# FREDZEL2020/jittor-MYC-NeRFs

Measured on AMD Instinct MI355X. Metric: ray_samples_per_sec, higher is better.
Workload: dtype f32 (emulated: 3 x f16-split MFMA products, fp32 accumulate; fp32 VALU elsewhere); 1 GPU; TensorVMSplit 300^3 (16/48 comps, MLP_Fea 150-128-128-3), 800x800 rays x 512 samples/ray (BASELINE configs[1]); ONE frame per step at every N (N>1: split over the ranks, BASELINE configs[2]), 512-ray tiles round-robin, one RCCL all_gather of [4 cap] fp32 (rgb block + depth block, written in place by the render) + two strided un-permute copies; scene=synthetic scene A (SURVEY 8d), no alpha mask, white_bg, samples_per_ray=512, rays_per_rank=640000, tile=512, chunk=640000, alpha_mask=0, emulate_world=0, arith=f32

## Files before the change

jittor-myc-nerfs_amd/csrc/tvr_march.hip:

```cpp
#include <cstdlib>
#include "tvr_device.h"
#include "tvr_kernels.h"
#include "tvr_march_body.h"
#include "tvr_gradient.h"


template <bool DENSE, bool LDSL>
__global__ __launch_bounds__(64 * MARCH_MAX_WAVES) void march_kernel(const SceneDev sc, const float *__restrict__ rays,
                                                                     const int n_rays, const int S, const int s_cap,
                                                                     const MarchSampling sm, const float eps_T,
                                                                     MarchOut mo, const tvr_dense_out dn)
{
    constexpr bool CP = false, VOL = false;
    const CpDev cp = {};
    const float *const dvol = nullptr;
#include "tvr_march_body.inc"
}

template <bool DENSE, bool PLAIN>
__global__ __launch_bounds__(64 * MARCH_VOL_WAVES, DENSE ? MARCH_VOL_OCC - 1 : MARCH_VOL_OCC) void march_vol_kernel(const SceneDev sc, const float *__restrict__ dvol, const float *__restrict__ rays,
                                                                         const int n_rays, const int S, const int s_cap, const MarchSampling sm, const float eps_T,
                                                                         MarchOut mo, const tvr_dense_out dn)
{
    static_assert(!(PLAIN && DENSE), "the plain form has no dense outputs");
    constexpr bool LDSL = false, CP = false, VOL = true;
    const CpDev cp = {};
#include "tvr_march_body.inc"
}

__global__ __launch_bounds__(256) void density_volume_kernel(const SceneDev sc, float *__restrict__ out)
{
    const long long gx1 = sc.grid[0] + 1, gy1 = sc.grid[1] + 1, gz1 = sc.grid[2] + 1;
    const long long t = (long long)blockIdx.x * blockDim.x + threadIdx.x;
    if (t >= gx1 * gy1 * gz1) return;
    const long long x = t % gx1, y = (t / gx1) % gy1, z = t / (gx1 * gy1);
    const float4 *P[3] = {sc.dplane[0] + (y * gx1 + x) * 4, sc.dplane[1] + (z * gx1 + x) * 4, sc.dplane[2] + (z * gy1 + y) * 4};
    const float4 *Ln[3] = {sc.dline[0] + z * 4, sc.dline[1] + y * 4, sc.dline[2] + x * 4};
    double acc = 0.0;
#pragma unroll
    for (int i = 0; i < 3; ++i) {
#pragma unroll
        for (int g = 0; g < 4; ++g) {
            const float4 p = P[i][g], l = Ln[i][g];
            acc = acc + (double)p.x * (double)l.x;
            acc = acc + (double)p.y * (double)l.y;
            acc = acc + (double)p.z * (double)l.z;
            acc = acc + (double)p.w * (double)l.w;
        }
    }
    out[t] = (float)acc;
}

hipError_t launch_density_volume(const SceneDev &sc, float *out, hipStream_t stream)
{
    const long long n = ((long long)sc.grid[0] + 1) * ((long long)sc.grid[1] + 1) * ((long long)sc.grid[2] + 1);
    hipLaunchKernelGGL(density_volume_kernel, dim3((unsigned)((n + 255) / 256)), dim3(256), 0, stream, sc, out);
    return hipGetLastError();
}

#define COMP_LANES 8
__global__ __launch_bounds__(256) void composite_kernel(const MarchOut mo, const int n_rays, const int white_bg,
                                                        float *__restrict__ rgb_out)
{
    const int t = blockIdx.x * blockDim.x + threadIdx.x;
    const int r = t / COMP_LANES, l = t % COMP_LANES;
    const bool live = r < n_rays;
    const unsigned base = live ? mo.ray_off[r] : 0u, cnt = live ? mo.ray_cnt[r] : 0u;
    float c0 = 0.f, c1 = 0.f, c2 = 0.f;
    unsigned i = l;
    for (; i + 3 * COMP_LANES < cnt; i += 4 * COMP_LANES) {
        const float4 e0 = mo.q_out[base + i], e1 = mo.q_out[base + i + COMP_LANES], e2 = mo.q_out[base + i + 2 * COMP_LANES],
                     e3 = mo.q_out[base + i + 3 * COMP_LANES];
        c0 = c0 + e0.w * e0.x; c1 = c1 + e0.w * e0.y; c2 = c2 + e0.w * e0.z;
        c0 = c0 + e1.w * e1.x; c1 = c1 + e1.w * e1.y; c2 = c2 + e1.w * e1.z;
        c0 = c0 + e2.w * e2.x; c1 = c1 + e2.w * e2.y; c2 = c2 + e2.w * e2.z;
        c0 = c0 + e3.w * e3.x; c1 = c1 + e3.w * e3.y; c2 = c2 + e3.w * e3.z;
    }
    for (; i < cnt; i += COMP_LANES) {
        const float4 e = mo.q_out[base + i];
        c0 = c0 + e.w * e.x;
        c1 = c1 + e.w * e.y;
        c2 = c2 + e.w * e.z;
    }
#pragma unroll
    for (int off = 1; off < COMP_LANES; off <<= 1) {
        c0 = c0 + __shfl_xor(c0, off);
        c1 = c1 + __shfl_xor(c1, off);
        c2 = c2 + __shfl_xor(c2, off);
    }
    if (!live || l != 0) return;
    if (mo.counter[2] != 0u) {
        const float qnan = __int_as_float(0x7fc00000);
        rgb_out[(size_t)r * 3 + 0] = qnan; rgb_out[(size_t)r * 3 + 1] = qnan; rgb_out[(size_t)r * 3 + 2] = qnan;
        mo.depth[r] = qnan;
        return;
    }
    const float acc = mo.acc[r];
    if (white_bg) {
        const float bg = 1.0f - acc;
        c0 = c0 + bg; c1 = c1 + bg; c2 = c2 + bg;
    }
    rgb_out[(size_t)r * 3 + 0] = clamp01(c0);
    rgb_out[(size_t)r * 3 + 1] = clamp01(c1);
    rgb_out[(size_t)r * 3 + 2] = clamp01(c2);
}

__global__ __launch_bounds__(256) void scatter_rgb_kernel(const MarchOut mo, const int S, float *__restrict__ rgb_dense)
{
    const unsigned n = *mo.counter;
    for (unsigned e = blockIdx.x * blockDim.x + threadIdx.x; e < n; e += gridDim.x * blockDim.x) {
        const float4 v = mo.q_out[e];
        const size_t q = ((size_t)mo.q_ray[e] * S + mo.q_j[e]) * 3;
        rgb_dense[q] = v.x; rgb_dense[q + 1] = v.y; rgb_dense[q + 2] = v.z;
    }
}

__global__ __launch_bounds__(256) void density_feature_kernel(const SceneDev sc, const float *__restrict__ xyz, const long long m,
                                                              float *__restrict__ out)
{
    const long long t = (long long)blockIdx.x * blockDim.x + threadIdx.x;
    const long long s = t >> 2;
    const int sub = threadIdx.x & 3;
    float part = 0.0f;
    if (s < m) {
        int i0[3];
        float w[3];
#pragma unroll
        for (int k = 0; k < 3; ++k) {
            const float f = unnorm(xyz[s * 3 + k], sc.gm1[k]);
            const float fl = floorf(fminf(fmaxf(f, -2.0f), sc.gm1[k] + 2.0f));
            i0[k] = (int)fl;
            w[k] = f - fl;
        }
        const float4 a = vm_term<4, true>(sc.dplane[0], sc.dline[0], sc.grid[0], sc.grid[1], sc.grid[2], i0[0], i0[1], i0[2], w[0], w[1], w[2], sub);
        const float4 b = vm_term<4, true>(sc.dplane[1], sc.dline[1], sc.grid[0], sc.grid[2], sc.grid[1], i0[0], i0[2], i0[1], w[0], w[2], w[1], sub);
        const float4 c = vm_term<4, true>(sc.dplane[2], sc.dline[2], sc.grid[1], sc.grid[2], sc.grid[0], i0[1], i0[2], i0[0], w[1], w[2], w[0], sub);
        part = ((a.x + a.y) + (a.z + a.w)) + ((b.x + b.y) + (b.z + b.w)) + ((c.x + c.y) + (c.z + c.w));
    }
    part += __shfl_xor(part, 1);
    part += __shfl_xor(part, 2);
    if (s < m && sub == 0) out[s] = part;
}

__global__ __launch_bounds__(256) void density_gradient_kernel(const SceneDev sc, const float *__restrict__ xyz, const long long m, const float3 h, const float3 inv2h,
                                                               float *__restrict__ sigma_feature, float *__restrict__ grad)
{
    const long long t = (long long)blockIdx.x * blockDim.x + threadIdx.x;
    const long long s = t >> 2;
    const int sub = threadIdx.x & 3;
    float f[7];
#pragma unroll
    for (int j = 0; j < 7; ++j) f[j] = 0.0f;
    if (s < m) vm_grad_point(sc, xyz[s * 3], xyz[s * 3 + 1], xyz[s * 3 + 2], h, sub, f);
#pragma unroll
    for (int j = 0; j < 7; ++j) {
        f[j] += __shfl_xor(f[j], 1);
        f[j] += __shfl_xor(f[j], 2);
    }
    if (s < m && sub == 0) {
        if (sigma_feature) sigma_feature[s] = f[0];
        grad[s * 3 + 0] = (f[1] - f[2]) * inv2h.x;
        grad[s * 3 + 1] = (f[3] - f[4]) * inv2h.y;
        grad[s * 3 + 2] = (f[5] - f[6]) * inv2h.z;
    }
}

__global__ __launch_bounds__(256) void alpha_sample_kernel(const SceneDev sc, const float *__restrict__ xyz, const long long m,
                                                           float *__restrict__ out)
{
    const long long s = (long long)blockIdx.x * blockDim.x + threadIdx.x;
    if (s >= m) return;
    const float p[3] = {xyz[s * 3], xyz[s * 3 + 1], xyz[s * 3 + 2]};
    out[s] = alpha_lookup(sc, p);
}

__global__ __launch_bounds__(256) void alpha_bits_kernel(const float *__restrict__ vol, const long long n, unsigned *__restrict__ bits)
{
    const long long wd = (long long)blockIdx.x * blockDim.x + threadIdx.x;
    if (wd * 32 >= n) return;
    unsigned v = 0u;
    for (int b = 0; b < 32; ++b) {
        const long long i = wd * 32 + b;
        if (i < n && vol[i] > 0.0f) v |= 1u << b;
    }
    bits[wd] = v;
}

hipError_t launch_alpha_bits(const float *vol, long long n, unsigned *bits, hipStream_t stream)
{
    const long long words = (n + 31) / 32;
    hipLaunchKernelGGL(alpha_bits_kernel, dim3((unsigned)((words + 255) / 256)), dim3(256), 0, stream, vol, n, bits);
    return hipGetLastError();
}

template <bool DENSE, bool LDSL>
static hipError_t launch_march_t(const SceneDev &sc, const float *rays, int n_rays, int S, const MarchSampling &sm, float eps_T, const MarchOut &mo,
                                 const tvr_dense_out &dn, int waves, size_t lds, unsigned grid, hipStream_t stream)
{
    hipError_t rc = hipFuncSetAttribute((const void *)march_kernel<DENSE, LDSL>, hipFuncAttributeMaxDynamicSharedMemorySize, (int)lds);
    if (rc != hipSuccess) return rc;
    hipLaunchKernelGGL((march_kernel<DENSE, LDSL>), dim3(grid), dim3(64 * waves), lds, stream, sc, rays, n_rays, S, S, sm, eps_T, mo, dn);
    return hipGetLastError();
}

static int device_cu_count()
{
    static int cus = 0;
    if (cus == 0) {
        int dev = 0, n = 0;
        if (hipGetDevice(&dev) == hipSuccess && hipDeviceGetAttribute(&n, hipDeviceAttributeMultiprocessorCount, dev) == hipSuccess && n > 0) cus = n;
        else cus = 256;
    }
    return cus;
}

int march_cu_count() { return device_cu_count(); }

static hipError_t launch_march_vol(const SceneDev &sc, const float *dvol, const float *rays, int n_rays, int S, const MarchSampling &sm, float eps_T, const MarchOut &mo,
                                   const tvr_dense_out *dense, hipStream_t stream)
{
    const int groups = MARCH_VOL_GROUPS;
    const size_t kLds = 160 * 1024 / (size_t)groups, per_wave = (size_t)S * 6, fixed = MARCH_HDR + 64;
    int waves = (int)((kLds - fixed) / per_wave);
    waves = waves >= MARCH_VOL_WAVES ? MARCH_VOL_WAVES : (waves >= 8 ? 8 : (waves >= 4 ? 4 : (waves >= 2 ? 2 : 1)));
    const size_t lds = fixed + (size_t)waves * per_wave;
    const int n_tiles = (n_rays + MARCH_TILE - 1) / MARCH_TILE;
    long long grid = (long long)device_cu_count() * groups * (MARCH_VOL_WAVES / waves);
    if (grid > n_tiles) grid = n_tiles;
    if (grid < 1) grid = 1;
    tvr_dense_out none = {};
    const tvr_dense_out &dn = dense ? *dense : none;
    const unsigned long long vol_bytes = 4ull * (unsigned long long)(sc.grid[0] + 1) * (unsigned long long)(sc.grid[1] + 1) * (unsigned long long)(sc.grid[2] + 1);
    const bool plain = !dense && sc.avol == nullptr && sm.zv == nullptr && mo.lam6 == nullptr && vol_bytes < (1ull << 32);
    const void *fn = dense ? (const void *)march_vol_kernel<true, false> : (plain ? (const void *)march_vol_kernel<false, true> : (const void *)march_vol_kernel<false, false>);
    hipError_t rc = hipFuncSetAttribute(fn, hipFuncAttributeMaxDynamicSharedMemorySize, (int)lds);
    if (rc != hipSuccess) return rc;
    if (dense) hipLaunchKernelGGL((march_vol_kernel<true, false>), dim3((unsigned)grid), dim3(64 * waves), lds, stream, sc, dvol, rays, n_rays, S, S, sm, eps_T, mo, dn);
    else if (plain) hipLaunchKernelGGL((march_vol_kernel<false, true>), dim3((unsigned)grid), dim3(64 * waves), lds, stream, sc, dvol, rays, n_rays, S, S, sm, eps_T, mo, dn);
    else hipLaunchKernelGGL((march_vol_kernel<false, false>), dim3((unsigned)grid), dim3(64 * waves), lds, stream, sc, dvol, rays, n_rays, S, S, sm, eps_T, mo, dn);
    return hipGetLastError();
}

hipError_t launch_march(const SceneDev &sc, const float *rays, int n_rays, int S, const MarchSampling &sm, float eps_T,
                        const MarchOut &mo, const tvr_dense_out *dense, hipStream_t stream, const float *dvol)
{
    if (dvol) return launch_march_vol(sc, dvol, rays, n_rays, S, sm, eps_T, mo, dense, stream);
    const size_t kLds = 160 * 1024, line_bytes = ((size_t)sc.grid[0] + sc.grid[1] + sc.grid[2] + 3) * 16 * MARCH_LSTRIDE, per_wave = (size_t)S * 6;
    bool ldsl = MARCH_HDR + line_bytes + 4 * per_wave + 64 <= kLds;
    const size_t fixed = MARCH_HDR + (ldsl ? line_bytes : 0) + 64;
    int waves = (int)((kLds - fixed) / per_wave);
    waves = waves >= 16 ? 16 : (waves >= 12 ? 12 : (waves >= 8 ? 8 : (waves >= 4 ? 4 : (waves >= 2 ? 2 : 1))));
    const size_t lds = fixed + (size_t)waves * per_wave;
    const int n_tiles = (n_rays + MARCH_TILE - 1) / MARCH_TILE;
    long long grid = (long long)device_cu_count() * (16 / waves > 0 ? 16 / waves : 1);
    if (grid > n_tiles) grid = n_tiles;
    if (grid < 1) grid = 1;
    tvr_dense_out none = {};
    const tvr_dense_out &dn = dense ? *dense : none;
    if (dense) return ldsl ? launch_march_t<true, true>(sc, rays, n_rays, S, sm, eps_T, mo, dn, waves, lds, (unsigned)grid, stream)
                           : launch_march_t<true, false>(sc, rays, n_rays, S, sm, eps_T, mo, dn, waves, lds, (unsigned)grid, stream);
    return ldsl ? launch_march_t<false, true>(sc, rays, n_rays, S, sm, eps_T, mo, dn, waves, lds, (unsigned)grid, stream)
                : launch_march_t<false, false>(sc, rays, n_rays, S, sm, eps_T, mo, dn, waves, lds, (unsigned)grid, stream);
}

hipError_t launch_composite(const MarchOut &mo, int n_rays, int white_bg, float *rgb, hipStream_t stream)
{
    const long long threads = (long long)n_rays * COMP_LANES;
    hipLaunchKernelGGL(composite_kernel, dim3((unsigned)((threads + 255) / 256)), dim3(256), 0, stream, mo, n_rays, white_bg, rgb);
    return hipGetLastError();
}

hipError_t launch_scatter_rgb(const MarchOut &mo, int S, float *rgb_dense, hipStream_t stream)
{
    hipLaunchKernelGGL(scatter_rgb_kernel, dim3(1024), dim3(256), 0, stream, mo, S, rgb_dense);
    return hipGetLastError();
}

hipError_t launch_density_feature(const SceneDev &sc, const float *xyz, long long m, float *out, hipStream_t stream)
{
    const long long blocks = (m * 4 + 255) / 256;
    hipLaunchKernelGGL(density_feature_kernel, dim3((unsigned)blocks), dim3(256), 0, stream, sc, xyz, m, out);
    return hipGetLastError();
}

hipError_t launch_density_gradient(const SceneDev &sc, const float *xyz, long long m, const float h[3], const float inv2h[3], float *sigma_feature, float *grad,
                                   hipStream_t stream)
{
    const long long blocks = (m * 4 + 255) / 256;
    hipLaunchKernelGGL(density_gradient_kernel, dim3((unsigned)blocks), dim3(256), 0, stream, sc, xyz, m, make_float3(h[0], h[1], h[2]),
                       make_float3(inv2h[0], inv2h[1], inv2h[2]), sigma_feature, grad);
    return hipGetLastError();
}

hipError_t launch_alpha_sample(const SceneDev &sc, const float *xyz, long long m, float *out, hipStream_t stream)
{
    hipLaunchKernelGGL(alpha_sample_kernel, dim3((unsigned)((m + 255) / 256)), dim3(256), 0, stream, sc, xyz, m, out);
    return hipGetLastError();
}
```

jittor-myc-nerfs_amd/csrc/tvr_march_body.h:

```cpp
#pragma once
#include "tvr_device.h"
#include "tvr_kernels.h"

#define MARCH_MAX_WAVES 16
#define MARCH_TILE 16
#define MARCH_SPIN_LIMIT (1u << 22)
#define MARCH_SLOTS 64u
#ifndef MARCH_CTR_WORD
#define MARCH_CTR_WORD 1
#endif
#ifndef MARCH_TAIL
#define MARCH_TAIL 4u
#endif
#ifndef MARCH_VOL_WAVES
#define MARCH_VOL_WAVES 16
#endif
#ifndef MARCH_VOL_GROUPS
#define MARCH_VOL_GROUPS 1
#endif
#ifndef MARCH_VOL_OCC
#define MARCH_VOL_OCC 8
#endif
#define MARCH_HDR 560
#ifndef MARCH_LSTRIDE
#define MARCH_LSTRIDE 4
#endif

__device__ __forceinline__ float4 vm_term_lds(const float4 *__restrict__ P, const float4 *Ls, int W, int x0, int y0, int l0,
                                              float wx, float wy, float wl, int sub)
{
    const float ux = 1.0f - wx, uy = 1.0f - wy, ul = 1.0f - wl;
    const int Wp = W + 1;
    const unsigned cell = __umul24((unsigned)y0, (unsigned)Wp) + (unsigned)x0;
    unsigned o0 = (cell << 6) + ((unsigned)sub << 4), o1 = o0 + ((unsigned)Wp << 6);
    asm volatile("" : "+v"(o0), "+v"(o1));
    const unsigned char *pb = (const unsigned char *)P;
    const float4 t00 = *(const float4 *)(pb + (size_t)o0), t01 = *(const float4 *)(pb + (size_t)o0 + 64);
    const float4 t10 = *(const float4 *)(pb + (size_t)o1), t11 = *(const float4 *)(pb + (size_t)o1 + 64);
    const float4 *q = Ls + l0 * MARCH_LSTRIDE + sub;
    const float4 l0v = q[0], l1v = q[MARCH_LSTRIDE];
    float4 p4 = f4_mul(ux * uy, t00);
    p4 = f4_fma(wx * uy, t01, p4);
    p4 = f4_fma(ux * wy, t10, p4);
    p4 = f4_fma(wx * wy, t11, p4);
    float4 q4 = f4_mul(ul, l0v);
    q4 = f4_fma(wl, l1v, q4);
    return make_float4(p4.x * q4.x, p4.y * q4.y, p4.z * q4.z, p4.w * q4.w);
}

__device__ __forceinline__ float cp_density_quad(const SceneDev &sc, const CpDev &cp, int ix, int iy, int iz, float wx, float wy, float wz, int sub)
{
    const int tpt = cp.rd >> 2;
    const float4 *__restrict__ l0 = sc.dline[0] + (size_t)iz * tpt + sub;
    const float4 *__restrict__ l1 = sc.dline[1] + (size_t)iy * tpt + sub;
    const float4 *__restrict__ l2 = sc.dline[2] + (size_t)ix * tpt + sub;
    const float ux = 1.0f - wx, uy = 1.0f - wy, uz = 1.0f - wz;
    float part = 0.0f;
    for (int g = 0; g < tpt; g += 4) {
        const float4 a0 = l0[g], a1 = l0[g + tpt], b0 = l1[g], b1 = l1[g + tpt], c0 = l2[g], c1 = l2[g + tpt];
        const float4 a = f4_fma(wz, a1, f4_mul(uz, a0)), b = f4_fma(wy, b1, f4_mul(uy, b0)), c = f4_fma(wx, c1, f4_mul(ux, c0));
        const float tx = (a.x * b.x) * c.x, ty = (a.y * b.y) * c.y, tz = (a.z * b.z) * c.z, tw = (a.w * b.w) * c.w;
        part = part + ((tx + ty) + (tz + tw));
    }
    return part;
}

struct __attribute__((packed, aligned(4))) vol_pair { float a, b; };
__device__ __forceinline__ float vol_density(const float *__restrict__ D, int gx1, int gy1, int ix, int iy, int iz, float wx, float wy, float wz)
{
    const size_t sy = (size_t)gx1, sz = (size_t)gx1 * (size_t)gy1;
    const float *r = D + ((size_t)iz * sz + (size_t)iy * sy + (size_t)ix);
    const vol_pair p00 = *(const vol_pair *)r, p01 = *(const vol_pair *)(r + sy);
    const vol_pair p10 = *(const vol_pair *)(r + sz), p11 = *(const vol_pair *)(r + sz + sy);
    const float c00 = __builtin_fmaf(wx, p00.b - p00.a, p00.a), c01 = __builtin_fmaf(wx, p01.b - p01.a, p01.a);
    const float c10 = __builtin_fmaf(wx, p10.b - p10.a, p10.a), c11 = __builtin_fmaf(wx, p11.b - p11.a, p11.a);
    const float c0 = __builtin_fmaf(wy, c01 - c00, c00), c1 = __builtin_fmaf(wy, c11 - c10, c10);
    return __builtin_fmaf(wz, c1 - c0, c0);
}

constexpr bool PLAIN = false;

struct MarchVolArgs {
    SceneDev sc;
    const float *dvol, *rays;
    int n_rays, S, s_cap;
    MarchSampling sm;
    float eps_T;
    MarchOut mo;
    tvr_dense_out dn;
};
template <bool ON_DEMAND, typename T>
__device__ __forceinline__ T march_arg_now(const T &arg, unsigned offset)
{
#if defined(__HIP_DEVICE_COMPILE__)
    if constexpr (ON_DEMAND) {
        const __attribute__((address_space(4))) unsigned char *ka = (const __attribute__((address_space(4))) unsigned char *)__builtin_amdgcn_kernarg_segment_ptr();
        asm volatile("" : "+s"(ka));
        return *(const __attribute__((address_space(4))) T *)(ka + offset);
    }
#endif
    return arg;
}

__device__ __forceinline__ float vol_density32(const unsigned char *r00, const unsigned char *r01, const unsigned char *r10, const unsigned char *r11, unsigned gx1,
                                               unsigned gy1, int ix, int iy, int iz, float wx, float wy, float wz)
{
    const unsigned row = __umul24((unsigned)iz, gy1) + (unsigned)iy;
    unsigned o = (row * gx1 + (unsigned)ix) << 2;
    asm volatile("" : "+v"(o));
    const vol_pair p00 = *(const vol_pair *)(r00 + (size_t)o), p01 = *(const vol_pair *)(r01 + (size_t)o);
    const vol_pair p10 = *(const vol_pair *)(r10 + (size_t)o), p11 = *(const vol_pair *)(r11 + (size_t)o);
    const float c00 = __builtin_fmaf(wx, p00.b - p00.a, p00.a), c01 = __builtin_fmaf(wx, p01.b - p01.a, p01.a);
    const float c10 = __builtin_fmaf(wx, p10.b - p10.a, p10.a), c11 = __builtin_fmaf(wx, p11.b - p11.a, p11.a);
    const float c0 = __builtin_fmaf(wy, c01 - c00, c00), c1 = __builtin_fmaf(wy, c11 - c10, c10);
    return __builtin_fmaf(wz, c1 - c0, c0);
}

#ifndef MARCH_VOL_LEAN
#define MARCH_VOL_LEAN 1
#endif
__device__ __forceinline__ float march_expf(float x)
{
    const float p = x * 0x1.715476p+0f;
    const float r = __builtin_rintf(p);
    float lo = __builtin_fmaf(x, 0x1.715476p+0f, -p);
    lo = __builtin_fmaf(x, 0x1.4ae0bep-26f, lo);
    return __builtin_ldexpf(__builtin_amdgcn_exp2f((p - r) + lo), (int)r);
}
__device__ __forceinline__ float march_softplus(float x)
{
    if (x > 20.0f) return x;
    const float t = march_expf(x);
    const float u = 1.0f + t, d = u - 1.0f;
    const float rc = __builtin_amdgcn_rcpf(d);
    float q = t * rc;
    q = __builtin_fmaf(__builtin_fmaf(-d, q, t), rc, q);
    const float lg = __builtin_amdgcn_logf(u) * 0x1.62e430p-1f;
    return d == 0.0f ? t : lg * q;
}

#define MARCH_DPP_WAVE_SHR1 0x138
#define MARCH_DPP_SAME 0xE4
template <int CTRL, int ROWS>
__device__ __forceinline__ float march_dpp_mov(float old, float v)
{
    return __int_as_float(__builtin_amdgcn_update_dpp(__float_as_int(old), __float_as_int(v), CTRL, ROWS, 0xF, false));
}
template <int N>
__device__ __forceinline__ float march_up(float v)
{
    float t = march_dpp_mov<MARCH_DPP_WAVE_SHR1, 0xF>(1.0f, v);
#pragma unroll
    for (int i = 1; i < N; ++i) t = march_dpp_mov<MARCH_DPP_WAVE_SHR1, 0xF>(t, t);
    return t;
}
__device__ __forceinline__ void scan_mul_dpp(float &x, float &excl, float &last)
{
    x = x * march_up<1>(x);
    x = x * march_up<2>(x);
    x = x * march_up<4>(x);
    x = x * march_up<8>(x);
    {
        const auto q = __builtin_amdgcn_permlane16_swap(__float_as_uint(x), __float_as_uint(x), false, false);
        const auto s = __builtin_amdgcn_permlane32_swap(q[0], q[1], false, false);
        float t = march_dpp_mov<MARCH_DPP_SAME, 0x6>(1.0f, __uint_as_float(s[0]));
        t = march_dpp_mov<MARCH_DPP_SAME, 0x8>(t, __uint_as_float(q[0]));
        x = x * t;
    }
    {
        const auto h = __builtin_amdgcn_permlane32_swap(__float_as_uint(x), __float_as_uint(x), false, false);
        x = x * march_dpp_mov<MARCH_DPP_SAME, 0xC>(1.0f, __uint_as_float(h[0]));
    }
    excl = march_up<1>(x);
    last = __int_as_float(__builtin_amdgcn_readlane(__float_as_int(x), 63));
}
```

jittor-myc-nerfs_amd/csrc/tvr_march_body.inc:

```
    static_assert(!(CP && LDSL), "the CP lines (up to 96 channels) do not go through LDS");
    static_assert(!(VOL && (CP || LDSL)), "the baked volume replaces the factored evaluation: no lines in LDS, no CP lines");
    extern __shared__ __attribute__((aligned(16))) unsigned char lds_raw[];
    const int lane = threadIdx.x & 63;
    const int wave = __builtin_amdgcn_readfirstlane(threadIdx.x >> 6);
    const int n_waves = blockDim.x >> 6;
    unsigned *cursor = (unsigned *)lds_raw;
    const float4 *ls0 = (const float4 *)(lds_raw + MARCH_HDR);
    const int ln0 = LDSL ? (sc.grid[2] + 1) * MARCH_LSTRIDE : 0, ln1 = LDSL ? (sc.grid[1] + 1) * MARCH_LSTRIDE : 0, ln2 = LDSL ? (sc.grid[0] + 1) * MARCH_LSTRIDE : 0;
    const float4 *ls1 = ls0 + ln0, *ls2 = ls1 + ln1;
    float *bufw = (float *)(ls2 + ln2) + (size_t)wave * s_cap;
    unsigned short *bufj = (unsigned short *)((float *)(ls2 + ln2) + (size_t)n_waves * s_cap) + (size_t)wave * s_cap;
#ifdef TVR_MARCH_TIMELINE
    unsigned long long tl_chunks = 0ull, tl_rays = 0ull;
    if (mo.stats && threadIdx.x == 0) mo.stats[32 + 8 * blockIdx.x] = __builtin_amdgcn_s_memrealtime();
#endif
    if (threadIdx.x == 0) *cursor = 0u;
    unsigned long long *slots = (unsigned long long *)(lds_raw + 16);
    if (threadIdx.x < MARCH_SLOTS) slots[threadIdx.x] = 0ull;
    unsigned long long *gstat = (unsigned long long *)(lds_raw + 16 + 8 * MARCH_SLOTS);
    if (threadIdx.x < 3) gstat[threadIdx.x] = 0ull;
    if (LDSL) {
        float4 *dst = (float4 *)(lds_raw + MARCH_HDR);
        for (int i = threadIdx.x; i < (sc.grid[2] + 1) * 4; i += blockDim.x) dst[(i >> 2) * MARCH_LSTRIDE + (i & 3)] = sc.dline[0][i];
        for (int i = threadIdx.x; i < (sc.grid[1] + 1) * 4; i += blockDim.x) dst[ln0 + (i >> 2) * MARCH_LSTRIDE + (i & 3)] = sc.dline[1][i];
        for (int i = threadIdx.x; i < (sc.grid[0] + 1) * 4; i += blockDim.x) dst[ln0 + ln1 + (i >> 2) * MARCH_LSTRIDE + (i & 3)] = sc.dline[2][i];
    }
    __syncthreads();
#ifdef TVR_MARCH_TIMELINE
    if (mo.stats && threadIdx.x == 0) mo.stats[32 + 8 * blockIdx.x + 1] = __builtin_amdgcn_s_memrealtime();
#endif
    const int sub = lane & 3;
    const unsigned char *vrow[4] = {nullptr, nullptr, nullptr, nullptr};
    if constexpr (PLAIN) {
        const size_t vsy = (size_t)(sc.grid[0] + 1) * 4, vsz = vsy * (size_t)(sc.grid[1] + 1);
        vrow[0] = (const unsigned char *)dvol; vrow[1] = vrow[0] + vsy; vrow[2] = vrow[0] + vsz; vrow[3] = vrow[2] + vsy;
    }
    unsigned long long clk0 = 0ull, ref0 = 0ull;
    if (march_arg_now<PLAIN>(mo.stats, offsetof(MarchVolArgs, mo.stats)) && threadIdx.x == 0) { clk0 = __builtin_amdgcn_s_memtime(); ref0 = __builtin_amdgcn_s_memrealtime(); }

    unsigned long long st_eval = 0, st_bbox = 0, st_term = 0;
    int last_start = 0;

    for (;;) {
        unsigned ci = 0;
        if (lane == 0) ci = atomicAdd(cursor, 1u);
        ci = __builtin_amdgcn_readfirstlane(ci);
        int ray_start, ray_len;
        {
            const unsigned k = ci / MARCH_TILE, slot = k & (MARCH_SLOTS - 1u);
            if ((ci % MARCH_TILE) == 0u) {
                unsigned t = 0, len = MARCH_TILE;
                if (lane == 0) {
                    if ((long long)n_rays >= 8LL * MARCH_TILE * (long long)gridDim.x && (long long)last_start + 2LL * MARCH_TILE * (long long)gridDim.x >= (long long)n_rays)
                        len = MARCH_TAIL;
                    t = atomicAdd(march_arg_now<PLAIN>(mo.counter, offsetof(MarchVolArgs, mo.counter)) + MARCH_CTR_WORD, len);
                    const unsigned long long genw = (unsigned long long)(k + 1u) | (len == MARCH_TAIL ? 0x80000000ull : 0ull);
#ifdef TVR_FAULT_INJECT_MARCH
                    if (blockIdx.x == 0 && k == 3u) __hip_atomic_store(&slots[slot], ((unsigned long long)(k + 1u + MARCH_SLOTS) << 32) | t, __ATOMIC_RELEASE, __HIP_MEMORY_SCOPE_WORKGROUP);
                    else
#endif
                    __hip_atomic_store(&slots[slot], (genw << 32) | t, __ATOMIC_RELEASE, __HIP_MEMORY_SCOPE_WORKGROUP);
                }
                ray_start = (int)__builtin_amdgcn_readfirstlane(t);
                ray_len = (int)__builtin_amdgcn_readfirstlane(len);
            } else {
                unsigned long long v;
                unsigned spins = 0u, fault = 0u;
                for (;;) {
                    v = __hip_atomic_load(&slots[slot], __ATOMIC_ACQUIRE, __HIP_MEMORY_SCOPE_WORKGROUP);
                    const unsigned gen = (unsigned)(v >> 32) & 0x7fffffffu;
                    if (gen == k + 1u) break;
                    if (gen > k + 1u) { fault = 1u; break; }
                    if (++spins > MARCH_SPIN_LIMIT) { fault = 2u; break; }
                    __builtin_amdgcn_s_sleep(1);
                }
                if (fault) {
                    if (lane == 0) atomicOr(march_arg_now<PLAIN>(mo.counter, offsetof(MarchVolArgs, mo.counter)) + 2, fault);
                    break;
                }
                ray_start = (int)(unsigned)v;
                ray_len = (v >> 63) ? MARCH_TAIL : MARCH_TILE;
            }
        }
        if (ray_start >= n_rays) break;
        if ((int)(ci % MARCH_TILE) >= ray_len) continue;
        last_start = ray_start;
        const int ray = ray_start + (int)(ci % MARCH_TILE);
        if (ray >= n_rays) continue;
        const float *__restrict__ const rays_r = march_arg_now<PLAIN>(rays, offsetof(MarchVolArgs, rays));
        const float *const jit_r = march_arg_now<PLAIN>(sm.jitter, offsetof(MarchVolArgs, sm.jitter));
        float o[3], d[3];
#pragma unroll
        for (int k = 0; k < 3; ++k) {
            o[k] = rays_r[(size_t)ray * 6 + k];
            d[k] = rays_r[(size_t)ray * 6 + 3 + k];
        }
        const float tmin = ray_tmin(sc, o, d);
        const bool has_jit = jit_r != nullptr;
        const float u = has_jit ? jit_r[ray] : 0.0f;
        const float *__restrict__ zrow = (!PLAIN && sm.zv) ? sm.zv + (size_t)ray * S : nullptr;
        float lam6 = 1.0f;
        int n6 = 0;

        float T = 1.0f, acc_l = 0.0f, dep_l = 0.0f;
        int napp = 0;
        bool seen = false, terminated = false;
        int c = 0;
        for (; c * 64 < S; ++c) {
            const int j = c * 64 + lane;
            const bool inr = j < S;
            float fj = (float)j, fj1 = (float)(j + 1);
            if (has_jit) { fj = fj + u; fj1 = fj1 + u; }
            float z = tmin + sc.step * fj;
            float z1 = tmin + sc.step * fj1;
            if (zrow) {
                z = inr ? zrow[j] : 0.0f;
                z1 = (j < S - 1) ? zrow[j + 1] : z;
            }
            float p[3], n[3], f[3];
            bool bbox = inr;
#pragma unroll
            for (int k = 0; k < 3; ++k) {
                p[k] = o[k] + d[k] * z;
                bbox = bbox & !((sc.lo[k] > p[k]) | (p[k] > sc.hi[k]));
            }
            bool valid = bbox;
            if (!PLAIN && sc.avol != nullptr) {
                if (bbox) valid = sc.abits ? alpha_positive(sc, p) : (alpha_lookup(sc, p) > 0.0f);
            }
            int i0[3];
            float w[3];
#pragma unroll
            for (int k = 0; k < 3; ++k) {
                n[k] = (p[k] - sc.lo[k]) * sc.inv[k] - 1.0f;
                f[k] = unnorm(n[k], sc.gm1[k]);
                const float fl = floorf(f[k]);
                i0[k] = (int)fl;
                w[k] = f[k] - fl;
            }
            if constexpr (PLAIN) asm volatile("" : "+v"(i0[0]), "+v"(i0[1]), "+v"(i0[2]), "+v"(w[0]), "+v"(w[1]), "+v"(w[2]));
            const unsigned long long mb = __ballot(bbox), mv = __ballot(valid);
            if (DENSE) {
                const size_t q = (size_t)ray * S + j;
                if (inr) {
                    if (dn.z) dn.z[q] = z;
                    if (dn.valid) dn.valid[q] = valid;
                    if (dn.bbox_valid) dn.bbox_valid[q] = bbox;
                    if (dn.cell) { dn.cell[q * 3] = i0[0]; dn.cell[q * 3 + 1] = i0[1]; dn.cell[q * 3 + 2] = i0[2]; }
                }
            }
            st_bbox += __popcll(mb);
            if (mv == 0ull) {
                if (DENSE && inr) {
                    const size_t q = (size_t)ray * S + j;
                    if (dn.sigma_feature) dn.sigma_feature[q] = 0.f;
                    if (dn.sigma) dn.sigma[q] = 0.f;
                    if (dn.alpha) dn.alpha[q] = 0.f;
                    if (dn.weight) dn.weight[q] = 0.f;
                }
                if (mb == 0ull && seen && !DENSE) break;
                continue;
            }
            seen = true;
            st_eval += __popcll(mv);
#ifdef TVR_MARCH_TIMELINE
            tl_chunks++;
#endif

            float sf = 0.0f;
            if constexpr (VOL) {
                if constexpr (PLAIN) {
                    if (valid) sf = vol_density32(vrow[0], vrow[1], vrow[2], vrow[3], (unsigned)(sc.grid[0] + 1), (unsigned)(sc.grid[1] + 1), i0[0], i0[1], i0[2], w[0], w[1], w[2]);
                } else
                if (valid) sf = vol_density(dvol, sc.grid[0] + 1, sc.grid[1] + 1, i0[0], i0[1], i0[2], w[0], w[1], w[2]);
            } else {
#pragma unroll
                for (int k4 = 0; k4 < 4; ++k4) {
                    const bool v = quad_bcast_i((int)valid, k4) != 0;
                    if (__ballot(v) == 0ull) continue;
                    const int ix = quad_bcast_i(i0[0], k4), iy = quad_bcast_i(i0[1], k4), iz = quad_bcast_i(i0[2], k4);
                    const float wx = quad_bcast_f(w[0], k4), wy = quad_bcast_f(w[1], k4), wz = quad_bcast_f(w[2], k4);
                    float part = 0.0f;
                    if constexpr (CP) {
                        if (v) part = cp_density_quad(sc, cp, ix, iy, iz, wx, wy, wz, sub);
                    } else
                    if (v && LDSL) {
                        const float4 a = vm_term_lds(sc.dplane[0], ls0, sc.grid[0], ix, iy, iz, wx, wy, wz, sub);
                        const float4 b = vm_term_lds(sc.dplane[1], ls1, sc.grid[0], ix, iz, iy, wx, wz, wy, sub);
                        const float4 cc = vm_term_lds(sc.dplane[2], ls2, sc.grid[1], iy, iz, ix, wy, wz, wx, sub);
                        part = ((a.x + a.y) + (a.z + a.w)) + ((b.x + b.y) + (b.z + b.w)) + ((cc.x + cc.y) + (cc.z + cc.w));
                    } else if (v) {
                        const float4 a = vm_term<4, false>(sc.dplane[0], sc.dline[0], sc.grid[0], sc.grid[1], sc.grid[2], ix, iy, iz, wx, wy, wz, sub);
                        const float4 b = vm_term<4, false>(sc.dplane[1], sc.dline[1], sc.grid[0], sc.grid[2], sc.grid[1], ix, iz, iy, wx, wz, wy, sub);
                        const float4 cc = vm_term<4, false>(sc.dplane[2], sc.dline[2], sc.grid[1], sc.grid[2], sc.grid[0], iy, iz, ix, wy, wz, wx, sub);
                        part = ((a.x + a.y) + (a.z + a.w)) + ((b.x + b.y) + (b.z + b.w)) + ((cc.x + cc.y) + (cc.z + cc.w));
                    }
                    part += quad_perm_f<QUAD_XOR1>(part);
                    part += quad_perm_f<QUAD_XOR2>(part);
                    if (sub == k4) sf = part;
                }
            }

            float sigma = 0.0f;
            constexpr bool LEAN = VOL && MARCH_VOL_LEAN;
            if constexpr (LEAN) {
                if (valid) sigma = (sc.act == 0) ? march_softplus(sf + sc.shift) : fmaxf(sf, 0.0f);
            } else
            if (valid) sigma = (sc.act == 0) ? softplus_f(sf + sc.shift) : fmaxf(sf, 0.0f);
            float dist = (j < S - 1) ? (z1 - z) : 0.0f;
            dist = dist * sc.scale;
            const float alpha = 1.0f - (LEAN ? march_expf(-sigma * dist) : expf(-sigma * dist));
            const float fT = (1.0f - alpha) + 1e-10f;
            if (!PLAIN && mo.lam6) {
                float f6 = inr ? (1.0f - alpha) + 1e-6f : 1.0f;
#pragma unroll
                for (int off = 32; off > 0; off >>= 1) f6 = f6 * __shfl_xor(f6, off);
                lam6 = lam6 * f6;
                n6 += min(64, S - c * 64);
            }
            float incl = fT, excl, last;
            if constexpr (VOL) {
                scan_mul_dpp(incl, excl, last);
            } else {
#pragma unroll
                for (int off = 1; off < 64; off <<= 1) {
                    const float t = __shfl_up(incl, off);
                    if (lane >= off) incl = incl * t;
                }
                excl = __shfl_up(incl, 1);
                if (lane == 0) excl = 1.0f;
            }
            const float Tj = T * excl;
            const float wgt = alpha * Tj;
            acc_l += wgt;
            dep_l += wgt * z;
            const bool app = wgt > sc.thres;
            const unsigned long long ma = __ballot(app);
            if (ma) {
                const int pos = napp + __popcll(ma & ((1ull << lane) - 1ull));
                if (app) { bufw[pos] = wgt; bufj[pos] = (unsigned short)j; }
                napp += __popcll(ma);
            }
            if constexpr (VOL) T = T * last;
            else T = T * __shfl(incl, 63);
            if (DENSE && inr) {
                const size_t q = (size_t)ray * S + j;
                if (dn.sigma_feature) dn.sigma_feature[q] = valid ? sf : 0.f;
                if (dn.sigma) dn.sigma[q] = sigma;
                if (dn.alpha) dn.alpha[q] = alpha;
                if (dn.weight) dn.weight[q] = wgt;
            }
            if (T < eps_T) { terminated = true; ++c; break; }
        }
        if (DENSE) {
            for (int cc = c; cc * 64 < S; ++cc) {
                const int j = cc * 64 + lane;
                if (j < S) {
                    const size_t q = (size_t)ray * S + j;
                    const float fjj = has_jit ? ((float)j + u) : (float)j;
                    if (dn.z) dn.z[q] = zrow ? zrow[j] : tmin + sc.step * fjj;
                    if (dn.valid) dn.valid[q] = 0;
                    if (dn.bbox_valid) dn.bbox_valid[q] = 0;
                    if (dn.cell) { dn.cell[q * 3] = 0; dn.cell[q * 3 + 1] = 0; dn.cell[q * 3 + 2] = 0; }
                    if (dn.sigma_feature) dn.sigma_feature[q] = 0.f;
                    if (dn.sigma) dn.sigma[q] = 0.f;
                    if (dn.alpha) dn.alpha[q] = 0.f;
                    if (dn.weight) dn.weight[q] = 0.f;
                }
            }
        }
        st_term += terminated ? 1 : 0;
#ifdef TVR_MARCH_TIMELINE
        tl_rays++;
#endif

        const float acc = wave_sum(acc_l);
        const float dep = wave_sum(dep_l);
        const MarchOut mt = march_arg_now<PLAIN>(mo, offsetof(MarchVolArgs, mo));
        unsigned base = 0;
        if (lane == 0 && napp > 0) base = atomicAdd(mt.counter, (unsigned)napp);
        base = __shfl(base, 0);
        if (lane == 0) {
            mt.ray_off[ray] = base;
            mt.ray_cnt[ray] = (unsigned)napp;
            mt.acc[ray] = acc;
            mt.depth[ray] = dep + (1.0f - acc) * d[2];
            if (!PLAIN && mt.lam6) mt.lam6[ray] = lam6 * expf((float)(S - n6) * 9.5367386e-7f);
            if (DENSE) {
                if (dn.bg_weight) dn.bg_weight[ray] = T;
                if (dn.acc) dn.acc[ray] = acc;
                if (dn.t_min) dn.t_min[ray] = tmin;
            }
        }
        __builtin_amdgcn_fence(__ATOMIC_ACQ_REL, "wavefront");
        for (int i = lane; i < napp; i += 64) {
            const unsigned ej = bufj[i];
            float fj = (float)ej;
            if (has_jit) fj = fj + u;
            const float z = zrow ? zrow[ej] : tmin + sc.step * fj;
            float4 qv;
            qv.x = ((o[0] + d[0] * z) - sc.lo[0]) * sc.inv[0] - 1.0f;
            qv.y = ((o[1] + d[1] * z) - sc.lo[1]) * sc.inv[1] - 1.0f;
            qv.z = ((o[2] + d[2] * z) - sc.lo[2]) * sc.inv[2] - 1.0f;
            qv.w = bufw[i];
            mt.q_pos[base + i] = qv;
            mt.q_ray[base + i] = (unsigned)ray;
            if (mt.q_j) mt.q_j[base + i] = ej;
        }
        __builtin_amdgcn_fence(__ATOMIC_ACQ_REL, "wavefront");
    }
#ifdef TVR_MARCH_TIMELINE
    if (mo.stats && lane == 0) {
        const unsigned long long te = __builtin_amdgcn_s_memrealtime();
        atomicMin((unsigned long long *)&mo.stats[32 + 8 * blockIdx.x + 2], te);
        atomicMax((unsigned long long *)&mo.stats[32 + 8 * blockIdx.x + 3], te);
        atomicAdd((unsigned long long *)&mo.stats[32 + 8 * blockIdx.x + 4], tl_chunks);
        atomicAdd((unsigned long long *)&mo.stats[32 + 8 * blockIdx.x + 5], tl_rays);
    }
#endif
    unsigned long long *const stats_r = march_arg_now<PLAIN>(mo.stats, offsetof(MarchVolArgs, mo.stats));
    if (stats_r) {
        if (lane == 0) {
            atomicAdd(&gstat[0], st_eval);
            atomicAdd(&gstat[1], st_bbox);
            atomicAdd(&gstat[2], st_term);
        }
        __syncthreads();
        if (threadIdx.x == 0) {
            atomicAdd((unsigned long long *)&stats_r[TVR_STAT_SAMPLES_EVAL], gstat[0]);
            atomicAdd((unsigned long long *)&stats_r[TVR_STAT_SAMPLES_BBOX], gstat[1]);
            atomicAdd((unsigned long long *)&stats_r[TVR_STAT_RAYS_TERMINATED], gstat[2]);
            atomicAdd((unsigned long long *)&stats_r[TVR_STAT_MARCH_CLK], __builtin_amdgcn_s_memtime() - clk0);
            atomicAdd((unsigned long long *)&stats_r[TVR_STAT_MARCH_REF], __builtin_amdgcn_s_memrealtime() - ref0);
        }
    }
```

Baseline: 26.41 billion ray-samples/s.

## Batch march compaction output across up to eight rays per wave via LDS ring

In the volume march kernel, each wave now buffers the surviving samples of several rays in an LDS ring buffer, together with small per-ray records (origin, direction, tmin, jitter, ray id, offset). It flushes them with a single global atomicAdd on the sample counter and one coalesced write pass, instead of an atomic and a short scatter per ray. The aim is less atomic contention on the global counter and fewer partial-wave stores when rays have few surviving samples. In exchange the kernel uses more LDS per wave, which can lower the wave count, and the flush does an extra linear search over pending records for each sample.

```diff
diff --git a/jittor-myc-nerfs_amd/csrc/tvr_march.hip b/jittor-myc-nerfs_amd/csrc/tvr_march.hip
--- a/jittor-myc-nerfs_amd/csrc/tvr_march.hip
+++ b/jittor-myc-nerfs_amd/csrc/tvr_march.hip
@@ -17,13 +17,13 @@
 #include "tvr_march_body.inc"
 }
 
-template <bool DENSE, bool PLAIN>
+template <bool DENSE, bool PLAIN, bool BATCH>
 __global__ __launch_bounds__(64 * MARCH_VOL_WAVES, DENSE ? MARCH_VOL_OCC - 1 : MARCH_VOL_OCC) void march_vol_kernel(const SceneDev sc, const float *__restrict__ dvol, const float *__restrict__ rays,
                                                                          const int n_rays, const int S, const int s_cap, const MarchSampling sm, const float eps_T,
                                                                          MarchOut mo, const tvr_dense_out dn)
 {
     static_assert(!(PLAIN && DENSE), "the plain form has no dense outputs");
-    constexpr bool LDSL = false, CP = false, VOL = true;
+    constexpr bool LDSL = false, CP = false, VOL = true, MARCH_BATCH = BATCH;
     const CpDev cp = {};
 #include "tvr_march_body.inc"
 }
@@ -220,24 +220,35 @@
                                    const tvr_dense_out *dense, hipStream_t stream)
 {
     const int groups = MARCH_VOL_GROUPS;
-    const size_t kLds = 160 * 1024 / (size_t)groups, per_wave = (size_t)S * 6, fixed = MARCH_HDR + 64;
-    int waves = (int)((kLds - fixed) / per_wave);
-    waves = waves >= MARCH_VOL_WAVES ? MARCH_VOL_WAVES : (waves >= 8 ? 8 : (waves >= 4 ? 4 : (waves >= 2 ? 2 : 1)));
-    const size_t lds = fixed + (size_t)waves * per_wave;
+    const size_t kLds = 160 * 1024 / (size_t)groups, per_list = (size_t)S * 6, fixed = MARCH_HDR + 64;
     const int n_tiles = (n_rays + MARCH_TILE - 1) / MARCH_TILE;
-    long long grid = (long long)device_cu_count() * groups * (MARCH_VOL_WAVES / waves);
-    if (grid > n_tiles) grid = n_tiles;
-    if (grid < 1) grid = 1;
+    int waves = 1;
+    size_t lds = 0;
+    long long grid = 1;
+    auto shape = [&](size_t per_pend) {
+        const int w = (int)((kLds - fixed - (per_pend ? 16 : 0)) / (per_list + per_pend));
+        waves = w >= MARCH_VOL_WAVES ? MARCH_VOL_WAVES : (w >= 8 ? 8 : (w >= 4 ? 4 : (w >= 2 ? 2 : 1)));
+        lds = per_pend ? fixed + (((size_t)waves * per_list + 15) & ~(size_t)15) + (size_t)waves * per_pend : fixed + (size_t)waves * per_list;
+        grid = (long long)device_cu_count() * groups * (MARCH_VOL_WAVES / waves);
+        if (grid > n_tiles) grid = n_tiles;
+        if (grid < 1) grid = 1;
+    };
+    shape(0);
+    const bool batch = (long long)n_rays > grid * (long long)waves;
+    if (batch) shape((size_t)MARCH_PEND * MARCH_PEND_WORDS * 4);
     tvr_dense_out none = {};
     const tvr_dense_out &dn = dense ? *dense : none;
     const unsigned long long vol_bytes = 4ull * (unsigned long long)(sc.grid[0] + 1) * (unsigned long long)(sc.grid[1] + 1) * (unsigned long long)(sc.grid[2] + 1);
     const bool plain = !dense && sc.avol == nullptr && sm.zv == nullptr && mo.lam6 == nullptr && vol_bytes < (1ull << 32);
-    const void *fn = dense ? (const void *)march_vol_kernel<true, false> : (plain ? (const void *)march_vol_kernel<false, true> : (const void *)march_vol_kernel<false, false>);
-    hipError_t rc = hipFuncSetAttribute(fn, hipFuncAttributeMaxDynamicSharedMemorySize, (int)lds);
+    hipError_t rc = hipSuccess;
+    auto go = [&](auto kern) {
+        rc = hipFuncSetAttribute((const void *)kern, hipFuncAttributeMaxDynamicSharedMemorySize, (int)lds);
+        if (rc == hipSuccess) hipLaunchKernelGGL(kern, dim3((unsigned)grid), dim3(64 * waves), lds, stream, sc, dvol, rays, n_rays, S, S, sm, eps_T, mo, dn);
+    };
+    if (dense) batch ? go(march_vol_kernel<true, false, true>) : go(march_vol_kernel<true, false, false>);
+    else if (plain) batch ? go(march_vol_kernel<false, true, true>) : go(march_vol_kernel<false, true, false>);
+    else batch ? go(march_vol_kernel<false, false, true>) : go(march_vol_kernel<false, false, false>);
     if (rc != hipSuccess) return rc;
-    if (dense) hipLaunchKernelGGL((march_vol_kernel<true, false>), dim3((unsigned)grid), dim3(64 * waves), lds, stream, sc, dvol, rays, n_rays, S, S, sm, eps_T, mo, dn);
-    else if (plain) hipLaunchKernelGGL((march_vol_kernel<false, true>), dim3((unsigned)grid), dim3(64 * waves), lds, stream, sc, dvol, rays, n_rays, S, S, sm, eps_T, mo, dn);
-    else hipLaunchKernelGGL((march_vol_kernel<false, false>), dim3((unsigned)grid), dim3(64 * waves), lds, stream, sc, dvol, rays, n_rays, S, S, sm, eps_T, mo, dn);
     return hipGetLastError();
 }
 
diff --git a/jittor-myc-nerfs_amd/csrc/tvr_march_body.h b/jittor-myc-nerfs_amd/csrc/tvr_march_body.h
--- a/jittor-myc-nerfs_amd/csrc/tvr_march_body.h
+++ b/jittor-myc-nerfs_amd/csrc/tvr_march_body.h
@@ -80,6 +80,10 @@
 
 constexpr bool PLAIN = false;
 
+constexpr bool MARCH_BATCH = false;
+#define MARCH_PEND 8
+#define MARCH_PEND_WORDS 12
+
 struct MarchVolArgs {
     SceneDev sc;
     const float *dvol, *rays;
@@ -174,3 +178,43 @@
     excl = march_up<1>(x);
     last = __int_as_float(__builtin_amdgcn_readlane(__float_as_int(x), 63));
 }
+
+template <bool PLAIN_F>
+__device__ __forceinline__ void march_flush(const SceneDev &sc, const MarchSampling &sm, const MarchOut &mo, const int S, const int s_cap, const int lane, const float *bufw,
+                                            const unsigned short *bufj, const float *pend, int &ring_head, int &pend_total, int &n_pend)
+{
+    __builtin_amdgcn_fence(__ATOMIC_ACQ_REL, "wavefront");
+    const MarchOut mf = march_arg_now<PLAIN_F>(mo, offsetof(MarchVolArgs, mo));
+    const bool jit_f = march_arg_now<PLAIN_F>(sm.jitter, offsetof(MarchVolArgs, sm.jitter)) != nullptr;
+    const int f_total = __builtin_amdgcn_readfirstlane(pend_total), f_rays = __builtin_amdgcn_readfirstlane(n_pend), f_head = __builtin_amdgcn_readfirstlane(ring_head);
+    unsigned fbase = 0;
+    if (lane == 0) fbase = atomicAdd(mf.counter, (unsigned)f_total);
+    fbase = __builtin_amdgcn_readfirstlane(fbase);
+    if (lane < f_rays) mf.ray_off[__float_as_uint(pend[lane * MARCH_PEND_WORDS + 8])] = fbase + __float_as_uint(pend[lane * MARCH_PEND_WORDS + 9]);
+    for (int i = lane; i < f_total; i += 64) {
+        int k = 0;
+        for (int m = 1; m < f_rays; ++m) k += (unsigned)i >= __float_as_uint(pend[m * MARCH_PEND_WORDS + 9]) ? 1 : 0;
+        const float *rec = pend + k * MARCH_PEND_WORDS;
+        int rp = f_head + i;
+        if (rp >= s_cap) rp -= s_cap;
+        const unsigned ej = bufj[rp];
+        const unsigned eray = __float_as_uint(rec[8]);
+        float fj = (float)ej;
+        if (jit_f) fj = fj + rec[7];
+        const float *__restrict__ zr = (!PLAIN_F && sm.zv) ? sm.zv + (size_t)eray * S : nullptr;
+        const float z = zr ? zr[ej] : rec[6] + sc.step * fj;
+        float4 qv;
+        qv.x = ((rec[0] + rec[3] * z) - sc.lo[0]) * sc.inv[0] - 1.0f;
+        qv.y = ((rec[1] + rec[4] * z) - sc.lo[1]) * sc.inv[1] - 1.0f;
+        qv.z = ((rec[2] + rec[5] * z) - sc.lo[2]) * sc.inv[2] - 1.0f;
+        qv.w = bufw[rp];
+        mf.q_pos[fbase + i] = qv;
+        mf.q_ray[fbase + i] = eray;
+        if (mf.q_j) mf.q_j[fbase + i] = ej;
+    }
+    __builtin_amdgcn_fence(__ATOMIC_ACQ_REL, "wavefront");
+    ring_head = f_head + f_total >= s_cap ? f_head + f_total - s_cap : f_head + f_total;
+    pend_total = 0;
+    n_pend = 0;
+    asm volatile("" : "+v"(ring_head), "+v"(pend_total), "+v"(n_pend));
+}
diff --git a/jittor-myc-nerfs_amd/csrc/tvr_march_body.inc b/jittor-myc-nerfs_amd/csrc/tvr_march_body.inc
--- a/jittor-myc-nerfs_amd/csrc/tvr_march_body.inc
+++ b/jittor-myc-nerfs_amd/csrc/tvr_march_body.inc
@@ -11,7 +11,7 @@
     float *bufw = (float *)(ls2 + ln2) + (size_t)wave * s_cap;
     unsigned short *bufj = (unsigned short *)((float *)(ls2 + ln2) + (size_t)n_waves * s_cap) + (size_t)wave * s_cap;
 #ifdef TVR_MARCH_TIMELINE
-    unsigned long long tl_chunks = 0ull, tl_rays = 0ull;
+    unsigned long long tl_chunks = 0ull, tl_rays = 0ull, tl_resv = 0ull;
     if (mo.stats && threadIdx.x == 0) mo.stats[32 + 8 * blockIdx.x] = __builtin_amdgcn_s_memrealtime();
 #endif
     if (threadIdx.x == 0) *cursor = 0u;
@@ -40,6 +40,13 @@
 
     unsigned long long st_eval = 0, st_bbox = 0, st_term = 0;
     int last_start = 0;
+
+    int ring_head = 0, pend_total = 0, n_pend = 0;
+    float *pend = nullptr;
+    if constexpr (MARCH_BATCH) {
+        pend = (float *)(lds_raw + ((MARCH_HDR + (size_t)n_waves * s_cap * 6 + 15) & ~(size_t)15)) + (size_t)wave * (MARCH_PEND * MARCH_PEND_WORDS);
+        asm volatile("" : "+v"(ring_head), "+v"(pend_total), "+v"(n_pend));
+    }
 
     for (;;) {
         unsigned ci = 0;
@@ -106,7 +113,12 @@
         int napp = 0;
         bool seen = false, terminated = false;
         int c = 0;
+        bool make_room = false;
+        for (;;) {
         for (; c * 64 < S; ++c) {
+            if constexpr (MARCH_BATCH) {
+                if (__ballot(n_pend > 0 && (n_pend == MARCH_PEND || pend_total + napp + 64 > s_cap))) { make_room = true; break; }
+            }
             const int j = c * 64 + lane;
             const bool inr = j < S;
             float fj = (float)j, fj1 = (float)(j + 1);
@@ -236,6 +248,14 @@
             dep_l += wgt * z;
             const bool app = wgt > sc.thres;
             const unsigned long long ma = __ballot(app);
+            if constexpr (MARCH_BATCH) {
+                if (ma) {
+                    int pos = ring_head + pend_total + napp + __popcll(ma & ((1ull << lane) - 1ull));
+                    if (pos >= s_cap) pos -= s_cap;
+                    if (app) { bufw[pos] = wgt; bufj[pos] = (unsigned short)j; }
+                    napp += __popcll(ma);
+                }
+            } else
             if (ma) {
                 const int pos = napp + __popcll(ma & ((1ull << lane) - 1ull));
                 if (app) { bufw[pos] = wgt; bufj[pos] = (unsigned short)j; }
@@ -251,6 +271,13 @@
                 if (dn.weight) dn.weight[q] = wgt;
             }
             if (T < eps_T) { terminated = true; ++c; break; }
+        }
+        if (!make_room) break;
+#ifdef TVR_MARCH_TIMELINE
+        tl_resv++;
+#endif
+        if constexpr (MARCH_BATCH) march_flush<PLAIN>(sc, sm, mo, S, s_cap, lane, bufw, bufj, pend, ring_head, pend_total, n_pend);
+        make_room = false;
         }
         if (DENSE) {
             for (int cc = c; cc * 64 < S; ++cc) {
@@ -277,7 +304,37 @@
         const float acc = wave_sum(acc_l);
         const float dep = wave_sum(dep_l);
         const MarchOut mt = march_arg_now<PLAIN>(mo, offsetof(MarchVolArgs, mo));
+        if constexpr (MARCH_BATCH) {
+            if (lane == 0) {
+                if (napp == 0) mt.ray_off[ray] = 0u;
+                mt.ray_cnt[ray] = (unsigned)napp;
+                mt.acc[ray] = acc;
+                mt.depth[ray] = dep + (1.0f - acc) * d[2];
+                if (!PLAIN && mt.lam6) mt.lam6[ray] = lam6 * expf((float)(S - n6) * 9.5367386e-7f);
+                if (DENSE) {
+                    if (dn.bg_weight) dn.bg_weight[ray] = T;
+                    if (dn.acc) dn.acc[ray] = acc;
+                    if (dn.t_min) dn.t_min[ray] = tmin;
+                }
+            }
+            if (napp > 0) {
+                if (lane == 0) {
+                    float *rec = pend + n_pend * MARCH_PEND_WORDS;
+                    rec[0] = o[0]; rec[1] = o[1]; rec[2] = o[2];
+                    rec[3] = d[0]; rec[4] = d[1]; rec[5] = d[2];
+                    rec[6] = tmin; rec[7] = u;
+                    rec[8] = __uint_as_float((unsigned)ray); rec[9] = __uint_as_float((unsigned)pend_total);
+                }
+                pend_total += napp;
+                ++n_pend;
+                asm volatile("" : "+v"(pend_total), "+v"(n_pend));
+            }
+            continue;
+        }
         unsigned base = 0;
+#ifdef TVR_MARCH_TIMELINE
+        if (napp > 0) tl_resv++;
+#endif
         if (lane == 0 && napp > 0) base = atomicAdd(mt.counter, (unsigned)napp);
         base = __shfl(base, 0);
         if (lane == 0) {
@@ -309,13 +366,19 @@
         }
         __builtin_amdgcn_fence(__ATOMIC_ACQ_REL, "wavefront");
     }
+    if constexpr (MARCH_BATCH) {
+#ifdef TVR_MARCH_TIMELINE
+        if (__ballot(n_pend > 0)) tl_resv++;
+#endif
+        if (__ballot(n_pend > 0)) march_flush<PLAIN>(sc, sm, mo, S, s_cap, lane, bufw, bufj, pend, ring_head, pend_total, n_pend);
+    }
 #ifdef TVR_MARCH_TIMELINE
     if (mo.stats && lane == 0) {
         const unsigned long long te = __builtin_amdgcn_s_memrealtime();
         atomicMin((unsigned long long *)&mo.stats[32 + 8 * blockIdx.x + 2], te);
         atomicMax((unsigned long long *)&mo.stats[32 + 8 * blockIdx.x + 3], te);
         atomicAdd((unsigned long long *)&mo.stats[32 + 8 * blockIdx.x + 4], tl_chunks);
-        atomicAdd((unsigned long long *)&mo.stats[32 + 8 * blockIdx.x + 5], tl_rays);
+        atomicAdd((unsigned long long *)&mo.stats[32 + 8 * blockIdx.x + 5], tl_rays | (tl_resv << 32));
     }
 #endif
     unsigned long long *const stats_r = march_arg_now<PLAIN>(mo.stats, offsetof(MarchVolArgs, mo.stats));
```

Result: faster. 28.30 billion ray-samples/s, median of 6 (+7.1%).
